# tobiasleibner/dune-hdd

Hardware: NVIDIA B200
Metric: assembled DoFs/s + CG solve s (SWIPDG p1, 16M cells) (higher is better)
Workload: dtype f64

## Files before the change

### dune_hdd_b200/csrc/multigrid.cu

```cuda
#include <algorithm>
#include <climits>
#include <cmath>
#include <cstdio>
#include <cstdlib>
#include <cstring>
#include <initializer_list>
#include <ctime>

#include "handles.hpp"
#include "reduce.cuh"

namespace hdd {

namespace {

constexpr int kMgThreads = 256;
constexpr int kMaxCoarse = 400;
constexpr double kOmega = 0.8;

inline int blocks_for(int64_t n) { return int((n + kMgThreads - 1) / kMgThreads); }

struct Rows {
  int64_t beg, cnt;
};

__device__ __forceinline__ void load_neigh4(const int32_t* neigh, int k, int* nb) {
  const int4 v = __ldg(reinterpret_cast<const int4*>(neigh) + k);
  nb[0] = v.x; nb[1] = v.y; nb[2] = v.z; nb[3] = v.w;
}

__global__ void k_struct_cells(const int32_t* __restrict__ cv, int32_t n_cells, int nx, int ny, int32_t* __restrict__ cell_v0,
                               int32_t* __restrict__ lex_cell, int32_t* flag) {
  const int c = blockIdx.x * blockDim.x + threadIdx.x;
  if (c >= n_cells) return;
  const int4 v = __ldg(reinterpret_cast<const int4*>(cv) + c);
  const int nx1 = nx + 1;
  const int cx = v.x % nx1, cy = v.x / nx1;
  if (v.x < 0 || cx >= nx || cy >= ny || v.y != v.x + 1 || v.z != v.x + nx1 || v.w != v.x + nx1 + 1) {
    atomicOr(flag, 1);
    return;
  }
  cell_v0[c] = v.x;
  lex_cell[cx + nx * cy] = c;
}

__global__ void k_struct_triangles(const int32_t* __restrict__ cv, int32_t n_cells, int nx1, int64_t n_verts, int32_t* flag) {
  const int c = blockIdx.x * blockDim.x + threadIdx.x;
  if (c >= n_cells) return;
  int vx[3], vy[3];
  for (int i = 0; i < 3; ++i) {
    const int v = cv[size_t(3) * c + i];
    if (v < 0 || v >= n_verts) { atomicOr(flag, 1); return; }
    vx[i] = v % nx1;
    vy[i] = v / nx1;
  }
  for (int i = 0; i < 3; ++i) {
    const int j = (i + 1) % 3;
    if (abs(vx[i] - vx[j]) > 1 || abs(vy[i] - vy[j]) > 1) atomicOr(flag, 1);
  }
}

__global__ void k_struct_verts(const double* __restrict__ xy , int64_t v0, int64_t count, int nx,
                               const double* __restrict__ xs, const double* __restrict__ ys, int32_t* flag) {
  const int64_t t = int64_t(blockIdx.x) * blockDim.x + threadIdx.x;
  if (t >= count) return;
  const int64_t v = v0 + t;
  const int nx1 = nx + 1;
  const double2 p = __ldg(reinterpret_cast<const double2*>(xy) + v);
  if (p.x != __ldg(xs + v % nx1) || p.y != __ldg(ys + v / nx1)) atomicOr(flag, 2);
}

__global__ void k_struct_geo(const double* __restrict__ xs, const double* __restrict__ ys, int nx, int ny, double* __restrict__ tgeo) {
  const int t = blockIdx.x * blockDim.x + threadIdx.x;
  if (t >= nx + ny) return;
  double4* out = reinterpret_cast<double4*>(tgeo);
  if (t < nx) {
    const double x0 = xs[t], x1 = xs[t + 1];
    out[t] = make_double4(x0, x1 - x0, 1.0 / (x1 - x0), 0.0);
  } else {
    const int r = t - nx;
    const double y0 = ys[r], y1 = ys[r + 1];
    out[t] = make_double4(y0, y1 - y0, 1.0 / (y1 - y0), 0.0);
  }
}

__global__ void __launch_bounds__(kMgThreads)
    k_vertex_galerkin(MeshView m, const double* __restrict__ vals, const int32_t* __restrict__ cell_v0,
                      const int32_t* __restrict__ lex_cell, int nx, int ny, Rows rg, double* __restrict__ S) {
  const int64_t nv = int64_t(nx + 1) * (ny + 1);
  const int64_t tid = int64_t(blockIdx.x) * blockDim.x + threadIdx.x;
  if (tid >= rg.cnt) return;
  const int64_t v = rg.beg + tid;
  const int nx1 = nx + 1;
  const int ix = int(v % nx1), iy = int(v / nx1);
  double acc[9];
#pragma unroll
  for (int e = 0; e < 9; ++e) acc[e] = 0.0;
#pragma unroll
  for (int b = 0; b < 2; ++b)
#pragma unroll
    for (int a = 0; a < 2; ++a) {
      const int cx = ix - 1 + a, cy = iy - 1 + b;
      if (cx < 0 || cy < 0 || cx >= nx || cy >= ny) continue;
      const int c = __ldg(lex_cell + cx + nx * cy);
      const int k = c - m.own0;
      if (c < 0 || k < 0 || k >= m.n_own) continue;
      const int i = (1 - a) + 2 * (1 - b);
      int nb[4];
      load_neigh4(m.neigh, k, nb);
      const int nblk = block_count<4>(nb);
      const double* row = vals + __ldg(m.blk_start + k) * 16 + int64_t(i) * nblk * 4;
#pragma unroll
      for (int t = 0; t < 5; ++t) {
        const int cell = t == 0 ? c : nb[t - 1];
        if (cell < 0) continue;
        const int slot = block_slot<4>(c, nb, cell);
        const int v0 = __ldg(cell_v0 + cell);
        const int jx = v0 % nx1 - ix, jy = v0 / nx1 - iy;
#pragma unroll
        for (int j = 0; j < 4; ++j) {
          const int dx = jx + (j & 1), dy = jy + (j >> 1);
          if (dx < -1 || dx > 1 || dy < -1 || dy > 1) continue;
          acc[(dy + 1) * 3 + dx + 1] += __ldg(row + slot * 4 + j);
        }
      }
    }
#pragma unroll
  for (int e = 0; e < 9; ++e) S[e * nv + v] = acc[e];
}

__global__ void k_twist_vector(const int* done, const double* __restrict__ b0, int nx, Rows rg, double* __restrict__ b1) {
  if (done && *done) return;
  const int64_t tid = int64_t(blockIdx.x) * blockDim.x + threadIdx.x;
  if (tid >= rg.cnt) return;
  const int64_t v = rg.beg + tid;
  const int nx1 = nx + 1;
  b1[v] = ((int(v % nx1) + int(v / nx1)) & 1) ? -b0[v] : b0[v];
}

__global__ void __launch_bounds__(kMgThreads)
    k_rap(const double* __restrict__ Sf, int64_t hf, int nxf, int nyf, int twist_h1, Rows rg, double* __restrict__ Sc, int64_t hc) {
  const int nxc = nxf / 2, nyc = nyf / 2;
  const int64_t nvc = int64_t(nxc + 1) * (nyc + 1), nvf = int64_t(nxf + 1) * (nyf + 1);
  const int64_t tid = int64_t(blockIdx.x) * blockDim.x + threadIdx.x;
  if (tid >= rg.cnt) return;
  const int twist = twist_h1 && blockIdx.y == 1;
  Sf += int64_t(blockIdx.y) * hf;
  Sc += int64_t(blockIdx.y) * hc;
  const int64_t I = rg.beg + tid;
  const int IX = int(I % (nxc + 1)), IY = int(I / (nxc + 1));
  double acc[9];
#pragma unroll
  for (int e = 0; e < 9; ++e) acc[e] = 0.0;
  for (int dy = -1; dy <= 1; ++dy)
    for (int dx = -1; dx <= 1; ++dx) {
      const int fx = 2 * IX + dx, fy = 2 * IY + dy;
      if (fx < 0 || fy < 0 || fx > nxf || fy > nyf) continue;
      const double wd = (dx == 0 ? 1.0 : 0.5) * (dy == 0 ? 1.0 : 0.5);
      const int64_t i = fx + int64_t(nxf + 1) * fy;
      for (int ey = -1; ey <= 1; ++ey)
        for (int ex = -1; ex <= 1; ++ex) {
          const int jx = fx + ex, jy = fy + ey;
          if (jx < 0 || jy < 0 || jx > nxf || jy > nyf) continue;
          double s = wd * __ldg(Sf + ((ey + 1) * 3 + ex + 1) * nvf + i);
          if (twist && ((ex + ey) & 1)) s = -s;
#pragma unroll
          for (int Dy = -1; Dy <= 1; ++Dy) {
            const int py = dy + ey - 2 * Dy;
            if (py < -1 || py > 1 || IY + Dy < 0 || IY + Dy > nyc) continue;
#pragma unroll
            for (int Dx = -1; Dx <= 1; ++Dx) {
              const int px = dx + ex - 2 * Dx;
              if (px < -1 || px > 1 || IX + Dx < 0 || IX + Dx > nxc) continue;
              acc[(Dy + 1) * 3 + Dx + 1] += s * (px == 0 ? 1.0 : 0.5) * (py == 0 ? 1.0 : 0.5);
            }
          }
        }
    }
#pragma unroll
  for (int e = 0; e < 9; ++e) Sc[e * nvc + I] = acc[e];
}

__global__ void __launch_bounds__(kMgThreads)
    k_mg_pre(const int* done, const double* __restrict__ S, const double* __restrict__ dinv, int nx, int ny, Rows rg,
             const double* __restrict__ b, double* __restrict__ x, double* __restrict__ r) {
  if (done && *done) return;
  const int nx1 = nx + 1;
  const int64_t nv = int64_t(nx1) * (ny + 1);
  const int64_t tid = int64_t(blockIdx.x) * blockDim.x + threadIdx.x;
  if (tid >= rg.cnt) return;
  const int64_t hv = int64_t(blockIdx.y) * nv;
  S += 9 * hv; dinv += hv; b += hv; x += hv; r += hv;
  const int64_t i = rg.beg + tid;
  const int ix = int(i % nx1), iy = int(i / nx1);
  double ax = 0.0;
#pragma unroll
  for (int ey = -1; ey <= 1; ++ey)
#pragma unroll
    for (int ex = -1; ex <= 1; ++ex) {
      const int jx = ix + ex, jy = iy + ey;
      if (jx < 0 || jy < 0 || jx > nx || jy > ny) continue;
      const int64_t j = i + ex + int64_t(ey) * nx1;
      const double xj = __ldg(dinv + j) * __ldg(b + j);
      ax = fma(__ldg(S + ((ey + 1) * 3 + ex + 1) * nv + i), xj, ax);
      if (ex == 0 && ey == 0) x[i] = xj;
    }
  r[i] = b[i] - ax;
}

__global__ void __launch_bounds__(kMgThreads)
    k_mg_restrict(const int* done, const double* __restrict__ r, int nxf, int nyf, Rows rg , double* __restrict__ bc) {
  if (done && *done) return;
  const int nxc = nxf / 2, nyc = nyf / 2;
  const int64_t tid = int64_t(blockIdx.x) * blockDim.x + threadIdx.x;
  if (tid >= rg.cnt) return;
  r += int64_t(blockIdx.y) * (int64_t(nxf + 1) * (nyf + 1));
  bc += int64_t(blockIdx.y) * (int64_t(nxc + 1) * (nyc + 1));
  const int64_t I = rg.beg + tid;
  const int IX = int(I % (nxc + 1)), IY = int(I / (nxc + 1));
  double s = 0.0;
#pragma unroll
  for (int dy = -1; dy <= 1; ++dy)
#pragma unroll
    for (int dx = -1; dx <= 1; ++dx) {
      const int fx = 2 * IX + dx, fy = 2 * IY + dy;
      if (fx < 0 || fy < 0 || fx > nxf || fy > nyf) continue;
      s = fma((dx == 0 ? 1.0 : 0.5) * (dy == 0 ? 1.0 : 0.5), __ldg(r + fx + int64_t(nxf + 1) * fy), s);
    }
  bc[I] = s;
}

__device__ __forceinline__ double mg_interp(const double* __restrict__ xc, int nxc1, int fx, int fy) {
  const int ox = fx & 1, oy = fy & 1;
  const int64_t I = (fx >> 1) + int64_t(nxc1) * (fy >> 1);
  double v = __ldg(xc + I);
  if (ox) v += __ldg(xc + I + 1);
  if (oy) {
    v += __ldg(xc + I + nxc1);
    if (ox) v += __ldg(xc + I + nxc1 + 1);
  }
  return v * (ox ? 0.5 : 1.0) * (oy ? 0.5 : 1.0);
}

__global__ void __launch_bounds__(kMgThreads)
    k_mg_prolong_add(const int* done, const double* __restrict__ xc, int nxf, int nyf, Rows rg , double* __restrict__ x) {
  if (done && *done) return;
  const int nxc = nxf / 2, nyc = nyf / 2;
  const int64_t tid = int64_t(blockIdx.x) * blockDim.x + threadIdx.x;
  if (tid >= rg.cnt) return;
  x += int64_t(blockIdx.y) * (int64_t(nxf + 1) * (nyf + 1));
  xc += int64_t(blockIdx.y) * (int64_t(nxc + 1) * (nyc + 1));
  const int64_t i = rg.beg + tid;
  x[i] += mg_interp(xc, nxc + 1, int(i % (nxf + 1)), int(i / (nxf + 1)));
}

__global__ void __launch_bounds__(kMgThreads)
    k_mg_post(const int* done, const double* __restrict__ S, const double* __restrict__ dinv, int nx, int ny, Rows rg,
              const double* __restrict__ b, const double* __restrict__ x, double* __restrict__ y) {
  if (done && *done) return;
  const int nx1 = nx + 1;
  const int64_t nv = int64_t(nx1) * (ny + 1);
  const int64_t tid = int64_t(blockIdx.x) * blockDim.x + threadIdx.x;
  if (tid >= rg.cnt) return;
  const int64_t hv = int64_t(blockIdx.y) * nv;
  S += 9 * hv; dinv += hv; b += hv; x += hv; y += hv;
  const int64_t i = rg.beg + tid;
  const int ix = int(i % nx1), iy = int(i / nx1);
  double ax = 0.0;
#pragma unroll
  for (int ey = -1; ey <= 1; ++ey)
#pragma unroll
    for (int ex = -1; ex <= 1; ++ex) {
      const int jx = ix + ex, jy = iy + ey;
      if (jx < 0 || jy < 0 || jx > nx || jy > ny) continue;
      ax = fma(__ldg(S + ((ey + 1) * 3 + ex + 1) * nv + i), __ldg(x + i + ex + int64_t(ey) * nx1), ax);
    }
  y[i] = fma(__ldg(dinv + i), b[i] - ax, x[i]);
}

__global__ void __launch_bounds__(kMgThreads)
    k_mg_up(const int* done, const double* __restrict__ S, const double* __restrict__ dinv, int nx, int ny, Rows rg,
            const double* __restrict__ b, const double* __restrict__ x, const double* __restrict__ xc, double* __restrict__ y) {
  if (done && *done) return;
  const int nx1 = nx + 1, nxc1 = nx / 2 + 1;
  const int64_t nv = int64_t(nx1) * (ny + 1);
  const int64_t tid = int64_t(blockIdx.x) * blockDim.x + threadIdx.x;
  if (tid >= rg.cnt) return;
  const int64_t hv = int64_t(blockIdx.y) * nv;
  S += 9 * hv; dinv += hv; b += hv; x += hv; y += hv;
  xc += int64_t(blockIdx.y) * (int64_t(nxc1) * (ny / 2 + 1));
  const int64_t i = rg.beg + tid;
  const int ix = int(i % nx1), iy = int(i / nx1);
  double ax = 0.0, xi = 0.0;
#pragma unroll
  for (int ey = -1; ey <= 1; ++ey)
#pragma unroll
    for (int ex = -1; ex <= 1; ++ex) {
      const int jx = ix + ex, jy = iy + ey;
      if (jx < 0 || jy < 0 || jx > nx || jy > ny) continue;
      const double xp = __ldg(x + i + ex + int64_t(ey) * nx1) + mg_interp(xc, nxc1, jx, jy);
      ax = fma(__ldg(S + ((ey + 1) * 3 + ex + 1) * nv + i), xp, ax);
      if (ex == 0 && ey == 0) xi = xp;
    }
  y[i] = fma(__ldg(dinv + i), b[i] - ax, xi);
}

__global__ void __launch_bounds__(kMgThreads)
    k_mg_pre2(const int* done, const double* __restrict__ S, const double* __restrict__ dinv, int nx, int ny, Rows rg,
              const double* __restrict__ b0, double* __restrict__ x0, double* __restrict__ r0) {
  if (done && *done) return;
  const int nx1 = nx + 1;
  const int64_t nv = int64_t(nx1) * (ny + 1);
  const int64_t tid = int64_t(blockIdx.x) * blockDim.x + threadIdx.x;
  if (tid >= rg.cnt) return;
  const double* b1 = b0 + nv;
  double* x1 = x0 + nv;
  double* r1 = r0 + nv;
  const int64_t i = rg.beg + tid;
  const int ix = int(i % nx1), iy = int(i / nx1);
  double a0 = 0.0, a1 = 0.0;
#pragma unroll
  for (int ey = -1; ey <= 1; ++ey)
#pragma unroll
    for (int ex = -1; ex <= 1; ++ex) {
      const int jx = ix + ex, jy = iy + ey;
      if (jx < 0 || jy < 0 || jx > nx || jy > ny) continue;
      const int64_t j = i + ex + int64_t(ey) * nx1;
      const double dj = __ldg(dinv + j);
      const double xj0 = dj * __ldg(b0 + j), xj1 = dj * __ldg(b1 + j);
      const double se = __ldg(S + ((ey + 1) * 3 + ex + 1) * nv + i);
      a0 = fma(se, xj0, a0);
      a1 = fma(((ex + ey) & 1) ? -se : se, xj1, a1);
      if (ex == 0 && ey == 0) { x0[i] = xj0; x1[i] = xj1; }
    }
  r0[i] = b0[i] - a0;
  r1[i] = b1[i] - a1;
}

__global__ void __launch_bounds__(kMgThreads)
    k_mg_post2(const int* done, const double* __restrict__ S, const double* __restrict__ dinv, int nx, int ny, Rows rg,
               const double* __restrict__ b0, const double* __restrict__ x0, double* __restrict__ y0) {
  if (done && *done) return;
  const int nx1 = nx + 1;
  const int64_t nv = int64_t(nx1) * (ny + 1);
  const int64_t tid = int64_t(blockIdx.x) * blockDim.x + threadIdx.x;
  if (tid >= rg.cnt) return;
  const double* b1 = b0 + nv;
  const double* x1 = x0 + nv;
  double* y1 = y0 + nv;
  const int64_t i = rg.beg + tid;
  const int ix = int(i % nx1), iy = int(i / nx1);
  double a0 = 0.0, a1 = 0.0;
#pragma unroll
  for (int ey = -1; ey <= 1; ++ey)
#pragma unroll
    for (int ex = -1; ex <= 1; ++ex) {
      const int jx = ix + ex, jy = iy + ey;
      if (jx < 0 || jy < 0 || jx > nx || jy > ny) continue;
      const int64_t j = i + ex + int64_t(ey) * nx1;
      const double se = __ldg(S + ((ey + 1) * 3 + ex + 1) * nv + i);
      a0 = fma(se, __ldg(x0 + j), a0);
      a1 = fma(((ex + ey) & 1) ? -se : se, __ldg(x1 + j), a1);
    }
  const double d = __ldg(dinv + i);
  y0[i] = fma(d, b0[i] - a0, x0[i]);
  y1[i] = fma(d, b1[i] - a1, x1[i]);
}

__global__ void k_mg_dinv(const double* __restrict__ S, int64_t nv, Rows rg, double* __restrict__ dinv) {
  const int64_t t = int64_t(blockIdx.x) * blockDim.x + threadIdx.x;
  const int64_t hv = int64_t(blockIdx.y) * nv;
  if (t < rg.cnt) dinv[hv + rg.beg + t] = kOmega / S[9 * hv + 4 * nv + rg.beg + t];
}

__global__ void k_mg_dense(const int* done, const double* __restrict__ Ainv, int n, const double* __restrict__ b,
                           double* __restrict__ x) {
  if (done && *done) return;
  const int i = blockIdx.x * (blockDim.x >> 5) + (threadIdx.x >> 5), lane = threadIdx.x & 31;
  if (i >= n) return;
  Ainv += size_t(blockIdx.y) * n * n;
  b += size_t(blockIdx.y) * n;
  x += size_t(blockIdx.y) * n;
  double s = 0.0;
  for (int j = lane; j < n; j += 32) s = fma(__ldg(Ainv + size_t(i) * n + j), __ldg(b + j), s);
  s = warp_sum(s);
  if (lane == 0) x[i] = s;
}

__global__ void __launch_bounds__(1024)
    k_dense_inverse(const double* __restrict__ S, int64_t hs , int nx, int ny,
                    int twist_h1, double* __restrict__ work, double* __restrict__ inv, int* flag) {
  __shared__ double col[kMaxCoarse];
  __shared__ double pivot_inv;
  const int nx1 = nx + 1, n = nx1 * (ny + 1);
  const int h = blockIdx.x;
  const bool twist = twist_h1 && h == 1;
  S += int64_t(h) * hs;
  double* A = work + size_t(h) * n * n;
  double* I = inv + size_t(h) * n * n;
  for (int t = threadIdx.x; t < n * n; t += blockDim.x) {
    const int i = t / n, j = t - i * n;
    const int ix = i % nx1, iy = i / nx1, jx = j % nx1, jy = j / nx1;
    const int ex = jx - ix, ey = jy - iy;
    double a = 0.0;
    if (ex >= -1 && ex <= 1 && ey >= -1 && ey <= 1) {
      a = S[int64_t((ey + 1) * 3 + ex + 1) * n + i];
      if (twist && ((ex + ey) & 1)) a = -a;
    }
    A[t] = a;
    I[t] = i == j ? 1.0 : 0.0;
  }
  __syncthreads();
  const int warp = threadIdx.x >> 5, lane = threadIdx.x & 31, n_warps = blockDim.x >> 5;
  for (int c = 0; c < n; ++c) {
    if (threadIdx.x == 0) {
      const double piv = A[size_t(c) * n + c];
      if (!(piv > 0.0)) atomicOr(flag, 1);
      pivot_inv = 1.0 / piv;
    }
    for (int i = threadIdx.x; i < n; i += blockDim.x) col[i] = i == c ? 0.0 : A[size_t(i) * n + c];
    __syncthreads();
    const double ip = pivot_inv;
    for (int j = threadIdx.x; j < n; j += blockDim.x) {
      A[size_t(c) * n + j] *= ip;
      I[size_t(c) * n + j] *= ip;
    }
    __syncthreads();
    for (int i = warp; i < n; i += n_warps) {
      const double f = col[i];
      if (f == 0.0) continue;
      for (int j = lane; j < n; j += 32) {
        A[size_t(i) * n + j] = fma(-f, A[size_t(c) * n + j], A[size_t(i) * n + j]);
        I[size_t(i) * n + j] = fma(-f, I[size_t(c) * n + j], I[size_t(i) * n + j]);
      }
    }
    __syncthreads();
  }
}

__global__ void __launch_bounds__(512)
    k_dense_inverse_banded(const double* __restrict__ S, int64_t hs, int nx, int ny, int twist_h1, double* __restrict__ work,
                           double* __restrict__ inv, int* flag) {
  extern __shared__ __align__(16) double Lb[];
  __shared__ double piv;
  const int nx1 = nx + 1, n = nx1 * (ny + 1), w = nx1 + 1, ld = w + 1;
  const int h = blockIdx.x;
  const bool twist = twist_h1 && h == 1;
  S += int64_t(h) * hs;
  double* Y = work + size_t(h) * n * n;
// ... 505 lines not shown
  const int sh = n_dist;
  d.own_lo = c0 >> sh;
  d.own_hi = last ? (ny >> sh) : (c1 >> sh) - 1;
  int res_lo = d.own_lo, res_hi = d.own_hi;
  for (int l = n_dist - 1; l >= 0; --l) {
    const int n = ny >> l;
    const int rr_lo = clip(2 * res_lo - 1, n), rr_hi = clip(2 * res_hi + 1, n);
    d.pre_lo[l] = std::min(d.pro_lo[l], rr_lo);
    d.pre_hi[l] = std::max(d.pro_hi[l], rr_hi);
    d.b_lo[l] = clip(d.pre_lo[l] - 1, n);
    d.b_hi[l] = clip(d.pre_hi[l] + 1, n);
    res_lo = d.b_lo[l];
    res_hi = d.b_hi[l];
  }
  d.ghost = std::max(c0 - d.b_lo[0], d.b_hi[0] - c1);
}

void mg_detect_structure(hdd_mesh* m, const double* xy_host, const double* xy_dev, int64_t v_begin, int64_t v_end,
                         const int32_t* cv_dev, int64_t n_verts) {
  m->sx = m->sy = 0;
  m->lx = m->ly = 0;
  int64_t nx1 = 1;
  while (nx1 < n_verts && xy_host[2 * nx1 + 1] == xy_host[1]) ++nx1;
  if (nx1 < 2 || n_verts % nx1 != 0) return;
  const int64_t nx = nx1 - 1, ny = n_verts / nx1 - 1;
  const bool simplex = m->kind == HDD_SIMPLEX2D;
  if (ny < 1 || (simplex ? 2 : 1) * nx * ny != m->n_global) return;
  cudaStream_t s = m->stream;
  std::vector<double> xs(static_cast<size_t>(nx1)), ys(static_cast<size_t>(ny + 1));
  for (int64_t i = 0; i < nx1; ++i) xs[size_t(i)] = xy_host[2 * i];
  for (int64_t j = 0; j <= ny; ++j) ys[size_t(j)] = xy_host[2 * j * nx1 + 1];
  DevBuf<double> d_xs, d_ys;
  d_xs.upload(xs.data(), xs.size(), s);
  d_ys.upload(ys.data(), ys.size(), s);
  DevBuf<int32_t> flag;
  flag.alloc(1);
  flag.zero(s);
  if (simplex) {
    k_struct_triangles<<<blocks_for(m->n_loc), kMgThreads, 0, s>>>(cv_dev, m->n_loc, int(nx1), n_verts, flag.p);
  } else {
    m->cell_v0.alloc(size_t(m->n_loc));
    m->lex_cell.alloc(size_t(m->n_global));
    HDD_CUDA(cudaMemsetAsync(m->lex_cell.p, 0xFF, size_t(m->n_global) * sizeof(int32_t), s));
    k_struct_cells<<<blocks_for(m->n_loc), kMgThreads, 0, s>>>(cv_dev, m->n_loc, int(nx), int(ny), m->cell_v0.p, m->lex_cell.p, flag.p);
    m->tgeo.alloc(4 * size_t(nx + ny));
    k_struct_geo<<<blocks_for(nx + ny), kMgThreads, 0, s>>>(d_xs.p, d_ys.p, int(nx), int(ny), m->tgeo.p);
  }
  k_struct_verts<<<blocks_for(v_end - v_begin), kMgThreads, 0, s>>>(xy_dev, v_begin, v_end - v_begin, int(nx), d_xs.p, d_ys.p, flag.p);
  count_launch(simplex ? 2 : 3);
  int32_t f = 0;
  HDD_CUDA(cudaMemcpyAsync(&f, flag.p, sizeof(f), cudaMemcpyDeviceToHost, s));
  HDD_CUDA(cudaStreamSynchronize(s));
  if (f != 0) {
    m->cell_v0.release();
    m->lex_cell.release();
    m->tgeo.release();
  } else if (simplex) {
    m->lx = int(nx);
    m->ly = int(ny);
  } else {
    m->sx = int(nx);
    m->sy = int(ny);
  }
}

static void build_hierarchies(hdd_swipdg* h, MgState& st) {
  hdd_mesh* m = h->mesh;
  cudaStream_t s = m->stream;
  const size_t nl = st.levels.size();
  const MgDist& d = st.dist;
  const int nd = d.on ? d.n_dist : 0;
  for (size_t l = 0; l + 1 < nl; ++l) {
    MgLevel& f = *st.levels[l];
    MgLevel& c = *st.levels[l + 1];
    Rows rc{0, c.nv};
    const int lc = int(l) + 1;
    const int nh = st.n_hier();
    if (lc < nd) {
      rc = row_range(c, d.b_lo[lc], d.b_hi[lc]);
    } else if (lc == nd && nd > 0) {
      HDD_CUDA(cudaMemsetAsync(c.S.p, 0, size_t(nh) * 9 * c.nv * sizeof(double), s));
      rc = row_range(c, d.own_lo, d.own_hi);
    }
    const bool shared = l == 0 && st.twisted0();
    k_rap<<<grid2(rc.cnt, nh), kMgThreads, 0, s>>>(f.S.p, shared ? 0 : 9 * f.nv, f.nx, f.ny, shared ? 1 : 0, rc, c.S.p, 9 * c.nv);
    count_launch();
    if (lc == nd && nd > 0) Nccl::get().all_reduce_sum(c.S.p, size_t(nh) * 9 * c.nv, m->comm, s);
  }
  for (size_t l = 0; l < nl; ++l) {
    MgLevel& L = *st.levels[l];
    const Rows r = int(l) < nd ? row_range(L, d.b_lo[l], d.b_hi[l]) : Rows{0, L.nv};
    k_mg_dinv<<<dim3(unsigned(blocks_for(r.cnt)), (l == 0 && st.twisted0()) ? 1u : unsigned(st.n_hier())), kMgThreads, 0, s>>>(L.S.p, L.nv, r, L.dinv.p);
    count_launch();
  }
  MgLevel& C = *st.levels.back();
  const char* type = st.type_name();
  if (C.nv > kMaxCoarse)
    HDD_THROW(HDD_ERR_REQUIREMENTS_NOT_MET, type << ": the " << st.nx << " x " << st.ny << " grid cannot be coarsened by halving down to at most "
                                                           << kMaxCoarse << " vertices (stuck at " << C.nx << " x " << C.ny << ")");
  const int n = int(C.nv);
  const bool shared = nl == 1 && st.twisted0();
  const size_t need = size_t(st.n_hier()) * n * n;
  if (st.coarse_inv.n < need) st.coarse_inv.alloc(need);
  if (st.coarse_work.n < need) st.coarse_work.alloc(need);
  if (!st.coarse_flag.p) st.coarse_flag.alloc(1);
  st.coarse_flag.zero(s);
  static const bool gauss_jordan = [] { const char* e = std::getenv("HDD_MG_COARSE_GJ"); return e && e[0] == '1'; }();
  const size_t band_bytes = size_t(n) * size_t(C.nx + 3) * sizeof(double);
  if (!gauss_jordan && band_bytes <= 200 * 1024 && n <= 512) {
    HDD_CUDA(cudaFuncSetAttribute(k_dense_inverse_banded, cudaFuncAttributeMaxDynamicSharedMemorySize, int(band_bytes)));
    k_dense_inverse_banded<<<st.n_hier(), 512, band_bytes, s>>>(C.S.p, shared ? 0 : int64_t(9) * n, C.nx, C.ny, shared ? 1 : 0,
                                                                st.coarse_work.p, st.coarse_inv.p, st.coarse_flag.p);
  } else {
    k_dense_inverse<<<st.n_hier(), 1024, 0, s>>>(C.S.p, shared ? 0 : int64_t(9) * n, C.nx, C.ny, shared ? 1 : 0, st.coarse_work.p,
                                                 st.coarse_inv.p, st.coarse_flag.p);
  }
  count_launch();
  int bad = 0;
  HDD_CUDA(cudaMemcpyAsync(&bad, st.coarse_flag.p, sizeof(int), cudaMemcpyDeviceToHost, s));
  HDD_CUDA(cudaStreamSynchronize(s));
  if (bad) HDD_THROW(HDD_ERR_REQUIREMENTS_NOT_MET, type << ": the coarsest operator is not positive definite");
}

constexpr int64_t kFusedUpMaxVerts = 1500000;

static void vcycle(hdd_mesh* m, MgState& st, const int* done, cudaStream_t s) {
  const int nl = int(st.levels.size());
  const MgDist& d = st.dist;
  const int nd = d.on ? d.n_dist : 0;
  const int nh = st.n_hier();
  SolvePhases& pt = phase_timer();
  for (int l = 0; l + 1 < nl; ++l) {
    MgLevel& L = *st.levels[size_t(l)];
    MgLevel& Cn = *st.levels[size_t(l) + 1];
    const Rows rp = l < nd ? row_range(L, d.pre_lo[l], d.pre_hi[l]) : Rows{0, L.nv};
    if (l == 0 && st.twisted0())
      k_mg_pre2<<<blocks_for(rp.cnt), kMgThreads, 0, s>>>(done, L.S.p, L.dinv.p, L.nx, L.ny, rp, L.b.p, L.x.p, L.r.p);
    else
      k_mg_pre<<<grid2(rp.cnt, nh), kMgThreads, 0, s>>>(done, L.S.p, L.dinv.p, L.nx, L.ny, rp, L.b.p, L.x.p, L.r.p);
    Rows rc{0, Cn.nv};
    if (l + 1 < nd) {
      rc = row_range(Cn, d.b_lo[l + 1], d.b_hi[l + 1]);
    } else if (l + 1 == nd && nd > 0) {
      HDD_CUDA(cudaMemsetAsync(Cn.b.p, 0, size_t(nh) * Cn.nv * sizeof(double), s));
      rc = row_range(Cn, d.own_lo, d.own_hi);
    }
    k_mg_restrict<<<grid2(rc.cnt, nh), kMgThreads, 0, s>>>(done, L.r.p, L.nx, L.ny, rc, Cn.b.p);
    count_launch(2);
    pt.mark(l == 0 ? "mg down level 0" : l < nd ? "mg down distributed 1.." : "mg down replicated", s);
    if (l + 1 == nd && nd > 0) {
      Nccl::get().all_reduce_sum(Cn.b.p, size_t(nh) * Cn.nv, m->comm, s);
      pt.mark("mg all-reduce coarse rhs", s);
    }
  }
  MgLevel& C = *st.levels.back();
  k_mg_dense<<<dim3(unsigned(int(C.nv) + 3) / 4, unsigned(nh)), 128, 0, s>>>(done, st.coarse_inv.p, int(C.nv), C.b.p, C.x.p);
  count_launch();
  pt.mark("mg dense", s);
  C.result = C.x.p;
  for (int l = nl - 2; l >= 0; --l) {
    MgLevel& L = *st.levels[size_t(l)];
    MgLevel& Cn = *st.levels[size_t(l) + 1];
    const Rows ru = l < nd ? row_range(L, d.up_lo[l], d.up_hi[l]) : Rows{0, L.nv};
    if (l > 0 && L.nv <= kFusedUpMaxVerts) {
      k_mg_up<<<grid2(ru.cnt, nh), kMgThreads, 0, s>>>(done, L.S.p, L.dinv.p, L.nx, L.ny, ru, L.b.p, L.x.p, Cn.result, L.y.p);
      count_launch();
    } else {
      const Rows rq = l < nd ? row_range(L, d.pro_lo[l], d.pro_hi[l]) : Rows{0, L.nv};
      k_mg_prolong_add<<<grid2(rq.cnt, nh), kMgThreads, 0, s>>>(done, Cn.result, L.nx, L.ny, rq, L.x.p);
      if (l == 0 && st.twisted0())
        k_mg_post2<<<blocks_for(ru.cnt), kMgThreads, 0, s>>>(done, L.S.p, L.dinv.p, L.nx, L.ny, ru, L.b.p, L.x.p, L.y.p);
      else
        k_mg_post<<<grid2(ru.cnt, nh), kMgThreads, 0, s>>>(done, L.S.p, L.dinv.p, L.nx, L.ny, ru, L.b.p, L.x.p, L.y.p);
      count_launch(2);
    }
    pt.mark(l == 0 ? "mg up level 0" : l < nd ? "mg up distributed 1.." : "mg up replicated", s);
    L.result = L.y.p;
  }
}

static void detect_strips(hdd_swipdg* h, MgState& st) {
  hdd_mesh* m = h->mesh;
  MgDist& d = st.dist;
  d.on = false;
  d.n_dist = 0;
  static const bool wanted = [] { const char* e = std::getenv("HDD_MG_DISTRIBUTED"); return !(e && e[0] == '0'); }();
  static const int cap = [] { const char* e = std::getenv("HDD_MG_DIST_LEVELS"); return e ? std::atoi(e) : kMaxDist; }();
  if (m->world <= 1) return;
  cudaStream_t s = m->stream;
  DevBuf<int> mm;
  const int init[2] = {INT32_MAX, -1};
  mm.upload(init, 2, s);
  const bool cube = m->kind == HDD_CUBE2D;
  if (m->n_own > 0) {
    if (cube)
      k_cell_row_range<<<blocks_for(m->n_own), kMgThreads, 0, s>>>(m->cell_v0.p + m->own0, m->n_own, st.nx, mm.p);
    else
      k_vertex_row_range<<<blocks_for(int64_t(3) * m->n_own), kMgThreads, 0, s>>>(m->cell_gv.p + size_t(3) * m->own0,
                                                                                 int64_t(3) * m->n_own, st.nx + 1, mm.p);
  }
  count_launch();
  int got[2] = {0, 0};
  HDD_CUDA(cudaMemcpyAsync(got, mm.p, sizeof(got), cudaMemcpyDeviceToHost, s));
  HDD_CUDA(cudaStreamSynchronize(s));
  const int c0 = got[0], c1 = cube ? got[1] + 1 : got[1];
  const bool band = m->n_own > 0 && int64_t(m->n_own) == int64_t(cube ? 1 : 2) * st.nx * (c1 - c0);
  std::vector<double> all(size_t(3) * m->world, 0.0);
  all[size_t(3) * m->rank] = c0;
  all[size_t(3) * m->rank + 1] = c1;
  all[size_t(3) * m->rank + 2] = band ? 1.0 : 0.0;
  DevBuf<double> buf;
  buf.upload(all.data(), all.size(), s);
  Nccl::get().all_reduce_sum(buf.p, all.size(), m->comm, s);
  HDD_CUDA(cudaMemcpyAsync(all.data(), buf.p, all.size() * sizeof(double), cudaMemcpyDeviceToHost, s));
  HDD_CUDA(cudaStreamSynchronize(s));
  if (!wanted) return;
  bool stacked = all[0] == 0.0 && all[size_t(3) * (m->world - 1) + 1] == double(st.ny);
  for (int r = 0; r < m->world; ++r) {
    stacked = stacked && all[size_t(3) * r + 2] == 1.0;
    if (r > 0) stacked = stacked && all[size_t(3) * r] == all[size_t(3) * (r - 1) + 1];
  }
  if (!stacked) return;
  int n_dist = 0;
  for (int n = std::min({cap, kMaxDist, int(st.levels.size()) - 1}); n >= 1 && n_dist == 0; --n) {
    bool ok = true;
    MgDist probe;
    mg_strip_plan(st.ny, 0, st.ny, n, probe);
    for (int r = 0; r < m->world && ok; ++r) {
      const int a = int(all[size_t(3) * r]), b = int(all[size_t(3) * r + 1]);
      MgDist pr;
      mg_strip_plan(st.ny, a, b, n, pr);
      ok = a % (1 << n) == 0 && (b % (1 << n) == 0 || b == st.ny) && (b - a) >= 2 * pr.ghost + 2;
    }
    if (ok) n_dist = n;
  }
  if (n_dist == 0) return;
  d.on = true;
  d.n_dist = n_dist;
  d.c0 = c0;
  d.c1 = c1;
  d.lower = m->rank > 0 ? m->rank - 1 : -1;
  d.upper = m->rank + 1 < m->world ? m->rank + 1 : -1;
  mg_strip_plan(st.ny, c0, c1, n_dist, d);
  const size_t rows = size_t(d.ghost) + 1;
  if (d.tmp_lo.n < rows * (size_t(st.nx) + 1)) {
    d.tmp_lo.alloc(rows * (size_t(st.nx) + 1));
    d.tmp_up.alloc(rows * (size_t(st.nx) + 1));
// ... 137 lines not shown
        kernel<<<blocks_for(m->n_verts_loc), kMgThreads, 0, s>>>(h->view(), vals, m->vptr.p, m->vdof.p, m->lvert_gid.p, m->cell_gv.p,
                                                                 m->n_verts_loc, st.nx, st.ny, f0.S.p);
        count_launch();
        if (m->world > 1) Nccl::get().all_reduce_sum(f0.S.p, size_t(9) * nv, m->comm, s);
        break;
      }
    }
  }
  HDD_CUDA(cudaGetLastError());
  phase_timer().mark("setup mg: level-0 operator", s);
  build_hierarchies(h, st);
  phase_timer().mark("setup mg: coarse operators", s);
  HDD_CUDA(cudaGetLastError());
}

void mg_apply(hdd_swipdg* h, const int* done, const double* r, double* z, double* p_init, double* partial, CgScalars* sc) {
  hdd_mesh* m = h->mesh;
  MgState& st = *h->mg;
  cudaStream_t s = m->stream;
  MgLevel& a = *st.levels[0];
  const bool multi = m->world > 1;
  const MgDist& d = st.dist;
  const int nx1 = st.nx + 1;
  double* b0 = a.b.p;
  double* b1 = a.b.p + a.nv;
  if (d.on) {
    const Rows mine{int64_t(d.c0) * nx1, int64_t(d.c1 - d.c0 + 1) * nx1};
    if (st.space == MgSpace::p1_lattice)
      k_dg_restrict_lattice<1><<<blocks_for(m->n_verts_loc), kMgThreads, 0, s>>>(done, r, m->vptr.p, m->vdof.p, m->lvert_gid.p,
                                                                                m->n_verts_loc, m->own0, m->n_own, b0);
    else
      k_dg_restrict<<<blocks_for(mine.cnt), kMgThreads, 0, s>>>(done, r, m->lex_cell.p, m->own0, m->n_own, st.nx, st.ny, mine, b0, nullptr);
    count_launch();
    phase_timer().mark("mg dg-restrict", s);
    const int g = d.ghost;
    const size_t cnt = size_t(g + 1) * nx1;
    Nccl& nc = Nccl::get();
    nc.group_start();
    if (d.upper >= 0) {
      nc.send(b0 + int64_t(d.c1 - g) * nx1, cnt, d.upper, m->comm, s);
      nc.recv(d.tmp_up.p, cnt, d.upper, m->comm, s);
    }
    if (d.lower >= 0) {
      nc.send(b0 + int64_t(d.c0) * nx1, cnt, d.lower, m->comm, s);
      nc.recv(d.tmp_lo.p, cnt, d.lower, m->comm, s);
    }
    nc.group_end();
    phase_timer().mark("mg ghost rows send/recv", s);
    const int lo_row = d.b_lo[0], hi_row = d.b_hi[0];
    k_ghost_unpack_twist<<<blocks_for(int64_t(hi_row - lo_row + 1) * nx1), kMgThreads, 0, s>>>(
        done, b0, b1, d.lower >= 0 ? d.tmp_lo.p : nullptr, d.upper >= 0 ? d.tmp_up.p : nullptr, st.nx, d.c0, d.c1, g, lo_row, hi_row);
    count_launch();
  } else {
    switch (st.space) {
      case MgSpace::q1_cube:
        k_dg_restrict<<<blocks_for(a.nv), kMgThreads, 0, s>>>(done, r, m->lex_cell.p, m->own0, m->n_own, st.nx, st.ny, Rows{0, a.nv}, b0,
                                                               multi ? nullptr : b1);
        count_launch();
        if (multi) {
          Nccl::get().all_reduce_sum(b0, size_t(a.nv), m->comm, s);
          k_twist_vector<<<blocks_for(a.nv), kMgThreads, 0, s>>>(done, b0, st.nx, Rows{0, a.nv}, b1);
          count_launch();
        }
        break;
      case MgSpace::q2_cube:
        k_dg_restrict_q2<<<blocks_for(a.nv), kMgThreads, 0, s>>>(done, r, m->lex_cell.p, m->own0, m->n_own, st.nx, st.ny, b0, b1);
        count_launch();
        if (multi) Nccl::get().all_reduce_sum(b0, size_t(2) * a.nv, m->comm, s);
        break;
      case MgSpace::p1_lattice:
      case MgSpace::p2_lattice: {
        const auto kernel = st.space == MgSpace::p1_lattice ? k_dg_restrict_lattice<1> : k_dg_restrict_lattice<2>;
        if (multi) HDD_CUDA(cudaMemsetAsync(b0, 0, size_t(a.nv) * sizeof(double), s));
        kernel<<<blocks_for(m->n_verts_loc), kMgThreads, 0, s>>>(done, r, m->vptr.p, m->vdof.p, m->lvert_gid.p, m->n_verts_loc, m->own0,
                                                                 m->n_own, b0);
        count_launch();
        if (multi) Nccl::get().all_reduce_sum(b0, size_t(a.nv), m->comm, s);
        break;
      }
    }
  }
  phase_timer().mark(d.on ? "mg ghost unpack" : "mg dg-restrict", s);
  if (st.levels.size() == 1) {
    k_mg_dense<<<dim3(unsigned(int(a.nv) + 3) / 4, unsigned(st.n_hier())), 128, 0, s>>>(done, st.coarse_inv.p, int(a.nv), a.b.p, a.x.p);
    count_launch();
    a.result = a.x.p;
  } else {
    vcycle(m, st, done, s);
  }
  const int grid = int(std::min<int64_t>((m->n_own + kMgThreads - 1) / kMgThreads, kMaxBlocks));
  switch (st.space) {
    case MgSpace::q1_cube:
      k_dg_prolong_dot<<<grid, kMgThreads, 0, s>>>(done, m->n_own, m->cell_v0.p + m->own0, st.nx, a.result, a.result + a.nv, r, z, p_init,
                                                   partial, sc);
      break;
    case MgSpace::q2_cube:
      k_dg_prolong_dot_q2<<<grid, kMgThreads, 0, s>>>(done, m->n_own, m->cell_v0.p + m->own0, st.nx, a.result, a.result + a.nv, r, z,
                                                      p_init, partial, sc);
      break;
    case MgSpace::p1_lattice:
    case MgSpace::p2_lattice: {
      const auto kernel = st.space == MgSpace::p1_lattice ? k_dg_prolong_dot_lattice<1> : k_dg_prolong_dot_lattice<2>;
      kernel<<<grid, kMgThreads, 0, s>>>(done, m->n_own, m->cell_gv.p + size_t(3) * m->own0, a.result, r, z, p_init, partial, sc);
      break;
    }
  }
  count_launch();
  phase_timer().mark("mg dg-prolong + r.z", s);
  HDD_CUDA(cudaGetLastError());
}

int mg_num_levels(const hdd_swipdg* h) { return h->mg ? int(h->mg->levels.size()) : 0; }

void mg_vertex_result(const hdd_swipdg* h, double* host) {
  const MgLevel& a = *h->mg->levels[0];
  HDD_CUDA(cudaMemcpyAsync(host, a.result, size_t(h->mg->n_hier()) * a.nv * sizeof(double), cudaMemcpyDeviceToHost,
                           h->mesh->stream));
}

}

extern "C" int hdd_mg_level_operator(const hdd_swipdg* h, int level, int hier, int* nx, int* ny, double* S_host) {
  return hdd::guarded([&] {
    if (!h) HDD_THROW(HDD_ERR_WRONG_INPUT, "discretization handle is NULL");
    const hdd::MgState* st = h->mg;
    if (!st) HDD_THROW(HDD_ERR_USING_THIS_WRONG, "no multigrid hierarchy: solve with 'cg.mg', 'cg.mg2' or 'cg.mg2.simplex' first");
    if (level < 0 || level >= int(st->levels.size()))
      HDD_THROW(HDD_ERR_WRONG_INPUT, "level " << level << " of " << st->levels.size());
    if (hier < 0 || hier >= st->n_hier()) HDD_THROW(HDD_ERR_WRONG_INPUT, "hierarchy " << hier << " of " << st->n_hier());
    if (level == 0 && hier == 1 && st->twisted0())
      HDD_THROW(HDD_ERR_WRONG_INPUT, "level 0 of the twisted hierarchy is C A_c C, read from the plain one's arrays");
    const hdd::MgLevel& L = *st->levels[size_t(level)];
    if (nx) *nx = L.nx;
    if (ny) *ny = L.ny;
    if (S_host) {
      h->mesh->set_device();
      cudaStream_t s = h->mesh->stream;
      HDD_CUDA(cudaMemcpyAsync(S_host, L.S.p + size_t(hier) * 9 * L.nv, size_t(9) * L.nv * sizeof(double),
                               cudaMemcpyDeviceToHost, s));
      HDD_CUDA(cudaStreamSynchronize(s));
    }
  });
}

extern "C" int hdd_mg_strip_plan(int ny, int c0, int c1, int n_dist, int* out) {
  if (!out || n_dist < 1 || n_dist > hdd::kMaxDist || c0 < 0 || c1 <= c0 || c1 > ny) return HDD_ERR_WRONG_INPUT;
  hdd::MgDist d;
  hdd::mg_strip_plan(ny, c0, c1, n_dist, d);
  for (int l = 0; l < n_dist; ++l) {
    const int v[8] = {d.pre_lo[l], d.pre_hi[l], d.b_lo[l], d.b_hi[l], d.up_lo[l], d.up_hi[l], d.pro_lo[l], d.pro_hi[l]};
    for (int k = 0; k < 8; ++k) out[8 * l + k] = v[k];
  }
  out[8 * n_dist] = d.own_lo;
  out[8 * n_dist + 1] = d.own_hi;
  out[8 * n_dist + 2] = d.ghost;
  return HDD_OK;
}
```

Before: 30.23 billion.

## Add shared-memory tiled multigrid down/up kernels and twin-hierarchy RAP and galerkin tweaks

```diff
diff --git a/dune_hdd_b200/csrc/multigrid.cu b/dune_hdd_b200/csrc/multigrid.cu
--- a/dune_hdd_b200/csrc/multigrid.cu
+++ b/dune_hdd_b200/csrc/multigrid.cu
@@ -17,6 +17,7 @@
 constexpr int kMgThreads = 256;
 constexpr int kMaxCoarse = 400;
 constexpr double kOmega = 0.8;
+constexpr int kDenseWarps = 2;
 
 inline int blocks_for(int64_t n) { return int((n + kMgThreads - 1) / kMgThreads); }
 
@@ -84,6 +85,37 @@
   }
 }
 
+__device__ __forceinline__ double4 pick_block(const double4 (&q)[5], int slot) {
+  double4 r = q[0];
+#pragma unroll
+  for (int k = 1; k < 5; ++k)
+    if (slot == k) r = q[k];
+  return r;
+}
+
+template <int JX, int JY>
+__device__ __forceinline__ void add_block(double (&acc)[9], const double4& q) {
+  const double bj[4] = {q.x, q.y, q.z, q.w};
+#pragma unroll
+  for (int j = 0; j < 4; ++j) {
+    const int dx = JX + (j & 1), dy = JY + (j >> 1);
+    if (dx < -1 || dx > 1 || dy < -1 || dy > 1) continue;
+    acc[(dy + 1) * 3 + dx + 1] += bj[j];
+  }
+}
+
+__device__ __forceinline__ void add_block(double (&acc)[9], const double4& q, int jx, int jy) {
+  switch ((jy + 2) * 4 + (jx + 2)) {
+#define HDD_ADD_BLOCK(k) \
+  case k: if (jx >= -2 && jx <= 1) add_block<(k) % 4 - 2, (k) / 4 - 2>(acc, q); break;
+    HDD_ADD_BLOCK(0) HDD_ADD_BLOCK(1) HDD_ADD_BLOCK(2) HDD_ADD_BLOCK(3) HDD_ADD_BLOCK(4) HDD_ADD_BLOCK(5)
+    HDD_ADD_BLOCK(6) HDD_ADD_BLOCK(7) HDD_ADD_BLOCK(8) HDD_ADD_BLOCK(9) HDD_ADD_BLOCK(10) HDD_ADD_BLOCK(11)
+    HDD_ADD_BLOCK(12) HDD_ADD_BLOCK(13) HDD_ADD_BLOCK(14) HDD_ADD_BLOCK(15)
+#undef HDD_ADD_BLOCK
+    default: break;
+  }
+}
+
 __global__ void __launch_bounds__(kMgThreads)
     k_vertex_galerkin(MeshView m, const double* __restrict__ vals, const int32_t* __restrict__ cell_v0,
                       const int32_t* __restrict__ lex_cell, int nx, int ny, Rows rg, double* __restrict__ S) {
@@ -109,20 +141,16 @@
       int nb[4];
       load_neigh4(m.neigh, k, nb);
       const int nblk = block_count<4>(nb);
-      const double* row = vals + __ldg(m.blk_start + k) * 16 + int64_t(i) * nblk * 4;
+      const double4* row = reinterpret_cast<const double4*>(vals + __ldg(m.blk_start + k) * 16 + int64_t(i) * nblk * 4);
+      double4 q[5];
+#pragma unroll
+      for (int t = 0; t < 5; ++t) q[t] = t < nblk ? row[t] : make_double4(0.0, 0.0, 0.0, 0.0);
 #pragma unroll
       for (int t = 0; t < 5; ++t) {
         const int cell = t == 0 ? c : nb[t - 1];
         if (cell < 0) continue;
-        const int slot = block_slot<4>(c, nb, cell);
         const int v0 = __ldg(cell_v0 + cell);
-        const int jx = v0 % nx1 - ix, jy = v0 / nx1 - iy;
-#pragma unroll
-        for (int j = 0; j < 4; ++j) {
-          const int dx = jx + (j & 1), dy = jy + (j >> 1);
-          if (dx < -1 || dx > 1 || dy < -1 || dy > 1) continue;
-          acc[(dy + 1) * 3 + dx + 1] += __ldg(row + slot * 4 + j);
-        }
+        add_block(acc, pick_block(q, block_slot<4>(c, nb, cell)), v0 % nx1 - ix, v0 / nx1 - iy);
       }
     }
 #pragma unroll
@@ -138,32 +166,38 @@
   b1[v] = ((int(v % nx1) + int(v / nx1)) & 1) ? -b0[v] : b0[v];
 }
 
-__global__ void __launch_bounds__(kMgThreads)
-    k_rap(const double* __restrict__ Sf, int64_t hf, int nxf, int nyf, int twist_h1, Rows rg, double* __restrict__ Sc, int64_t hc) {
+template <bool kTwin>
+__global__ void __launch_bounds__(kMgThreads)
+    k_rap(const double* __restrict__ Sf, int64_t hf, int nxf, int nyf, Rows rg, double* __restrict__ Sc, int64_t hc) {
+  constexpr int NH = kTwin ? 2 : 1;
   const int nxc = nxf / 2, nyc = nyf / 2;
   const int64_t nvc = int64_t(nxc + 1) * (nyc + 1), nvf = int64_t(nxf + 1) * (nyf + 1);
   const int64_t tid = int64_t(blockIdx.x) * blockDim.x + threadIdx.x;
   if (tid >= rg.cnt) return;
-  const int twist = twist_h1 && blockIdx.y == 1;
   Sf += int64_t(blockIdx.y) * hf;
   Sc += int64_t(blockIdx.y) * hc;
   const int64_t I = rg.beg + tid;
   const int IX = int(I % (nxc + 1)), IY = int(I / (nxc + 1));
-  double acc[9];
-#pragma unroll
-  for (int e = 0; e < 9; ++e) acc[e] = 0.0;
+  double acc[NH][9];
+#pragma unroll
+  for (int h = 0; h < NH; ++h)
+#pragma unroll
+    for (int e = 0; e < 9; ++e) acc[h][e] = 0.0;
+#pragma unroll
   for (int dy = -1; dy <= 1; ++dy)
+#pragma unroll
     for (int dx = -1; dx <= 1; ++dx) {
       const int fx = 2 * IX + dx, fy = 2 * IY + dy;
       if (fx < 0 || fy < 0 || fx > nxf || fy > nyf) continue;
       const double wd = (dx == 0 ? 1.0 : 0.5) * (dy == 0 ? 1.0 : 0.5);
       const int64_t i = fx + int64_t(nxf + 1) * fy;
+#pragma unroll
       for (int ey = -1; ey <= 1; ++ey)
+#pragma unroll
         for (int ex = -1; ex <= 1; ++ex) {
           const int jx = fx + ex, jy = fy + ey;
           if (jx < 0 || jy < 0 || jx > nxf || jy > nyf) continue;
-          double s = wd * __ldg(Sf + ((ey + 1) * 3 + ex + 1) * nvf + i);
-          if (twist && ((ex + ey) & 1)) s = -s;
+          const double s = wd * __ldg(Sf + ((ey + 1) * 3 + ex + 1) * nvf + i);
 #pragma unroll
           for (int Dy = -1; Dy <= 1; ++Dy) {
             const int py = dy + ey - 2 * Dy;
@@ -172,13 +206,19 @@
             for (int Dx = -1; Dx <= 1; ++Dx) {
               const int px = dx + ex - 2 * Dx;
               if (px < -1 || px > 1 || IX + Dx < 0 || IX + Dx > nxc) continue;
-              acc[(Dy + 1) * 3 + Dx + 1] += s * (px == 0 ? 1.0 : 0.5) * (py == 0 ? 1.0 : 0.5);
+#pragma unroll
+              for (int h = 0; h < NH; ++h) {
+                const double sh = (h == 1 && ((ex + ey) & 1)) ? -s : s;
+                acc[h][(Dy + 1) * 3 + Dx + 1] += sh * (px == 0 ? 1.0 : 0.5) * (py == 0 ? 1.0 : 0.5);
+              }
             }
           }
         }
     }
 #pragma unroll
-  for (int e = 0; e < 9; ++e) Sc[e * nvc + I] = acc[e];
+  for (int h = 0; h < NH; ++h)
+#pragma unroll
+    for (int e = 0; e < 9; ++e) Sc[h * hc + e * nvc + I] = acc[h][e];
 }
 
 __global__ void __launch_bounds__(kMgThreads)
@@ -337,6 +377,83 @@
   r1[i] = b1[i] - a1;
 }
 
+constexpr int kDnTx = 32, kDnTy = 8;
+static_assert(kDnTx * kDnTy == kMgThreads, "one thread per coarse vertex of the tile");
+
+template <bool kTwin>
+__global__ void __launch_bounds__(kMgThreads)
+    k_mg_down_tile(const int* done, const double* __restrict__ S, const double* __restrict__ dinv, int nx, int ny,
+                   const double* __restrict__ b, double* __restrict__ x, double* __restrict__ bc) {
+  if (done && *done) return;
+  constexpr int NH = kTwin ? 2 : 1, RX = 2 * kDnTx + 1, RY = 2 * kDnTy + 1, XX = RX + 2, XY = RY + 2;
+  __shared__ double xs[NH][XY][XX];
+  __shared__ double rs[NH][RY][RX];
+  const int nx1 = nx + 1, nxc = nx / 2, nyc = ny / 2;
+  const int64_t nv = int64_t(nx1) * (ny + 1), nvc = int64_t(nxc + 1) * (nyc + 1);
+  if (!kTwin) {
+    const int64_t z = blockIdx.z;
+    S += 9 * nv * z; dinv += nv * z; b += nv * z; x += nv * z; bc += nvc * z;
+  }
+  const int IX0 = blockIdx.x * kDnTx, IY0 = blockIdx.y * kDnTy;
+  for (int k = threadIdx.x; k < XX * XY; k += kMgThreads) {
+    const int hx = k % XX, hy = k / XX;
+    const int jx = 2 * IX0 - 2 + hx, jy = 2 * IY0 - 2 + hy;
+    if (jx < 0 || jy < 0 || jx > nx || jy > ny) continue;
+    const int64_t j = jx + int64_t(jy) * nx1;
+    const double dj = __ldg(dinv + j);
+    const bool own = hx >= 2 && hx < 2 + 2 * kDnTx && hy >= 2 && hy < 2 + 2 * kDnTy;
+#pragma unroll
+    for (int h = 0; h < NH; ++h) {
+      const double xj = dj * __ldg(b + h * nv + j);
+      xs[h][hy][hx] = xj;
+      if (own) x[h * nv + j] = xj;
+    }
+  }
+  __syncthreads();
+  for (int k = threadIdx.x; k < RX * RY; k += kMgThreads) {
+    const int hx = k % RX, hy = k / RX;
+    const int ix = 2 * IX0 - 1 + hx, iy = 2 * IY0 - 1 + hy;
+    if (ix < 0 || iy < 0 || ix > nx || iy > ny) continue;
+    const int64_t i = ix + int64_t(iy) * nx1;
+    double a[NH];
+#pragma unroll
+    for (int h = 0; h < NH; ++h) a[h] = 0.0;
+#pragma unroll
+    for (int ey = -1; ey <= 1; ++ey)
+#pragma unroll
+      for (int ex = -1; ex <= 1; ++ex) {
+        const int jx = ix + ex, jy = iy + ey;
+        if (jx < 0 || jy < 0 || jx > nx || jy > ny) continue;
+        const double se = __ldg(S + ((ey + 1) * 3 + ex + 1) * nv + i);
+#pragma unroll
+        for (int h = 0; h < NH; ++h)
+          a[h] = fma((h == 1 && ((ex + ey) & 1)) ? -se : se, xs[h][hy + 1 + ey][hx + 1 + ex], a[h]);
+      }
+#pragma unroll
+    for (int h = 0; h < NH; ++h) rs[h][hy][hx] = __ldg(b + h * nv + i) - a[h];
+  }
+  __syncthreads();
+  const int lx = threadIdx.x % kDnTx, ly = threadIdx.x / kDnTx;
+  const int IX = IX0 + lx, IY = IY0 + ly;
+  if (IX > nxc || IY > nyc) return;
+  double sum[NH];
+#pragma unroll
+  for (int h = 0; h < NH; ++h) sum[h] = 0.0;
+#pragma unroll
+  for (int dy = -1; dy <= 1; ++dy)
+#pragma unroll
+    for (int dx = -1; dx <= 1; ++dx) {
+      const int fx = 2 * IX + dx, fy = 2 * IY + dy;
+      if (fx < 0 || fy < 0 || fx > nx || fy > ny) continue;
+      const double w = (dx == 0 ? 1.0 : 0.5) * (dy == 0 ? 1.0 : 0.5);
+#pragma unroll
+      for (int h = 0; h < NH; ++h) sum[h] = fma(w, rs[h][2 * ly + 1 + dy][2 * lx + 1 + dx], sum[h]);
+    }
+  const int64_t I = IX + int64_t(nxc + 1) * IY;
+#pragma unroll
+  for (int h = 0; h < NH; ++h) bc[h * nvc + I] = sum[h];
+}
+
 __global__ void __launch_bounds__(kMgThreads)
     k_mg_post2(const int* done, const double* __restrict__ S, const double* __restrict__ dinv, int nx, int ny, Rows rg,
                const double* __restrict__ b0, const double* __restrict__ x0, double* __restrict__ y0) {
@@ -365,6 +482,55 @@
   const double d = __ldg(dinv + i);
   y0[i] = fma(d, b0[i] - a0, x0[i]);
   y1[i] = fma(d, b1[i] - a1, x1[i]);
+}
+
+constexpr int kUpTx = 64, kUpTy = 4;
+static_assert(kUpTx * kUpTy == kMgThreads, "one thread per tile vertex");
+
+template <bool kTwin>
+__global__ void __launch_bounds__(kMgThreads)
+    k_mg_up_tile(const int* done, const double* __restrict__ S, const double* __restrict__ dinv, int nx, int ny,
+                 const double* __restrict__ b, const double* __restrict__ x, const double* __restrict__ xc, double* __restrict__ y) {
+  if (done && *done) return;
+  constexpr int NH = kTwin ? 2 : 1, HX = kUpTx + 2, HY = kUpTy + 2;
+  __shared__ double xs[NH][HY][HX];
+  const int nx1 = nx + 1, nxc1 = nx / 2 + 1;
+  const int64_t nv = int64_t(nx1) * (ny + 1), nvc = int64_t(nxc1) * (ny / 2 + 1);
+  if (!kTwin) {
+    const int64_t z = blockIdx.z;
+    S += 9 * nv * z; dinv += nv * z; b += nv * z; x += nv * z; xc += nvc * z; y += nv * z;
+  }
+  const int tx0 = blockIdx.x * kUpTx, ty0 = blockIdx.y * kUpTy;
+  for (int k = threadIdx.x; k < HX * HY; k += kMgThreads) {
+    const int hx = k % HX, hy = k / HX;
+    const int jx = tx0 - 1 + hx, jy = ty0 - 1 + hy;
+    if (jx < 0 || jy < 0 || jx > nx || jy > ny) continue;
+    const int64_t j = jx + int64_t(jy) * nx1;
+#pragma unroll
+    for (int h = 0; h < NH; ++h) xs[h][hy][hx] = __ldg(x + h * nv + j) + mg_interp(xc + h * nvc, nxc1, jx, jy);
+  }
+  __syncthreads();
+  const int lx = threadIdx.x % kUpTx, ly = threadIdx.x / kUpTx;
+  const int ix = tx0 + lx, iy = ty0 + ly;
+  if (ix > nx || iy > ny) return;
+  const int64_t i = ix + int64_t(iy) * nx1;
+  double a[NH];
+#pragma unroll
+  for (int h = 0; h < NH; ++h) a[h] = 0.0;
+#pragma unroll
+  for (int ey = -1; ey <= 1; ++ey)
+#pragma unroll
+    for (int ex = -1; ex <= 1; ++ex) {
+      const int jx = ix + ex, jy = iy + ey;
+      if (jx < 0 || jy < 0 || jx > nx || jy > ny) continue;
+      const double se = __ldg(S + ((ey + 1) * 3 + ex + 1) * nv + i);
+#pragma unroll
+      for (int h = 0; h < NH; ++h)
+        a[h] = fma((h == 1 && ((ex + ey) & 1)) ? -se : se, xs[h][ly + 1 + ey][lx + 1 + ex], a[h]);
+    }
+  const double d = __ldg(dinv + i);
+#pragma unroll
+  for (int h = 0; h < NH; ++h) y[h * nv + i] = fma(d, b[h * nv + i] - a[h], xs[h][ly + 1][lx + 1]);
 }
 
 __global__ void k_mg_dinv(const double* __restrict__ S, int64_t nv, Rows rg, double* __restrict__ dinv) {
@@ -1036,8 +1202,10 @@
       HDD_CUDA(cudaMemsetAsync(c.S.p, 0, size_t(nh) * 9 * c.nv * sizeof(double), s));
       rc = row_range(c, d.own_lo, d.own_hi);
     }
-    const bool shared = l == 0 && st.twisted0();
-    k_rap<<<grid2(rc.cnt, nh), kMgThreads, 0, s>>>(f.S.p, shared ? 0 : 9 * f.nv, f.nx, f.ny, shared ? 1 : 0, rc, c.S.p, 9 * c.nv);
+    if (l == 0 && st.twisted0())
+      k_rap<true><<<grid2(rc.cnt, 1), kMgThreads, 0, s>>>(f.S.p, 0, f.nx, f.ny, rc, c.S.p, 9 * c.nv);
+    else
+      k_rap<false><<<grid2(rc.cnt, nh), kMgThreads, 0, s>>>(f.S.p, 9 * f.nv, f.nx, f.ny, rc, c.S.p, 9 * c.nv);
     count_launch();
     if (lc == nd && nd > 0) Nccl::get().all_reduce_sum(c.S.p, size_t(nh) * 9 * c.nv, m->comm, s);
   }
@@ -1088,6 +1256,17 @@
     MgLevel& L = *st.levels[size_t(l)];
     MgLevel& Cn = *st.levels[size_t(l) + 1];
     const Rows rp = l < nd ? row_range(L, d.pre_lo[l], d.pre_hi[l]) : Rows{0, L.nv};
+    if (m->world == 1) {
+      const bool twin = l == 0 && st.twisted0();
+      const dim3 tiles(unsigned((Cn.nx + kDnTx) / kDnTx), unsigned((Cn.ny + kDnTy) / kDnTy), twin ? 1u : unsigned(nh));
+      if (twin)
+        k_mg_down_tile<true><<<tiles, kMgThreads, 0, s>>>(done, L.S.p, L.dinv.p, L.nx, L.ny, L.b.p, L.x.p, Cn.b.p);
+      else
+        k_mg_down_tile<false><<<tiles, kMgThreads, 0, s>>>(done, L.S.p, L.dinv.p, L.nx, L.ny, L.b.p, L.x.p, Cn.b.p);
+      count_launch();
+      pt.mark(l == 0 ? "mg down level 0" : "mg down replicated", s);
+      continue;
+    }
     if (l == 0 && st.twisted0())
       k_mg_pre2<<<blocks_for(rp.cnt), kMgThreads, 0, s>>>(done, L.S.p, L.dinv.p, L.nx, L.ny, rp, L.b.p, L.x.p, L.r.p);
     else
@@ -1108,7 +1287,8 @@
     }
   }
   MgLevel& C = *st.levels.back();
-  k_mg_dense<<<dim3(unsigned(int(C.nv) + 3) / 4, unsigned(nh)), 128, 0, s>>>(done, st.coarse_inv.p, int(C.nv), C.b.p, C.x.p);
+  k_mg_dense<<<dim3(unsigned(int(C.nv) + kDenseWarps - 1) / kDenseWarps, unsigned(nh)), 32 * kDenseWarps, 0, s>>>(
+      done, st.coarse_inv.p, int(C.nv), C.b.p, C.x.p);
   count_launch();
   pt.mark("mg dense", s);
   C.result = C.x.p;
@@ -1116,7 +1296,15 @@
     MgLevel& L = *st.levels[size_t(l)];
     MgLevel& Cn = *st.levels[size_t(l) + 1];
     const Rows ru = l < nd ? row_range(L, d.up_lo[l], d.up_hi[l]) : Rows{0, L.nv};
-    if (l > 0 && L.nv <= kFusedUpMaxVerts) {
+    if (m->world == 1) {
+      const bool twin = l == 0 && st.twisted0();
+      const dim3 tiles(unsigned((L.nx + kUpTx) / kUpTx), unsigned((L.ny + kUpTy) / kUpTy), twin ? 1u : unsigned(nh));
+      if (twin)
+        k_mg_up_tile<true><<<tiles, kMgThreads, 0, s>>>(done, L.S.p, L.dinv.p, L.nx, L.ny, L.b.p, L.x.p, Cn.result, L.y.p);
+      else
+        k_mg_up_tile<false><<<tiles, kMgThreads, 0, s>>>(done, L.S.p, L.dinv.p, L.nx, L.ny, L.b.p, L.x.p, Cn.result, L.y.p);
+      count_launch();
+    } else if (l > 0 && L.nv <= kFusedUpMaxVerts) {
       k_mg_up<<<grid2(ru.cnt, nh), kMgThreads, 0, s>>>(done, L.S.p, L.dinv.p, L.nx, L.ny, ru, L.b.p, L.x.p, Cn.result, L.y.p);
       count_launch();
     } else {
@@ -1420,7 +1608,8 @@
   }
   phase_timer().mark(d.on ? "mg ghost unpack" : "mg dg-restrict", s);
   if (st.levels.size() == 1) {
-    k_mg_dense<<<dim3(unsigned(int(a.nv) + 3) / 4, unsigned(st.n_hier())), 128, 0, s>>>(done, st.coarse_inv.p, int(a.nv), a.b.p, a.x.p);
+    k_mg_dense<<<dim3(unsigned(int(a.nv) + kDenseWarps - 1) / kDenseWarps, unsigned(st.n_hier())), 32 * kDenseWarps, 0, s>>>(
+        done, st.coarse_inv.p, int(a.nv), a.b.p, a.x.p);
     count_launch();
     a.result = a.x.p;
   } else {
```

Result: slower. 29.51 billion, median of 6 (-2.4%).
